# stoyannk/voxels

Hardware: NVIDIA B200
Metric: Mvoxels/s polygonized (higher is better)
Workload: dtype int8 samples / fp32 vertices

## Files before the change

### voxels_b200/csrc/vxb_cell.h

```cpp
#pragma once
#include <stdint.h>

#if defined(__CUDACC__)
#define VXB_FN __device__ __forceinline__
#define VXB_FN_BIG __device__ __forceinline__
#define VXB_SQRT(x) __fsqrt_rn(x)
#define VXB_DIV(a, b) __fdiv_rn((a), (b))
#else
#include <cmath>
#define VXB_FN inline
#define VXB_FN_BIG inline
#define VXB_SQRT(x) std::sqrt(x)
#define VXB_DIV(a, b) ((a) / (b))
#endif

#define VXB_BLOCK 16
#define VXB_EMPTY_MATERIAL 255
#define VXB_NO_SLOT 0xF

enum { VXB_ZPOS = 0, VXB_YPOS = 1, VXB_XPOS = 2, VXB_ZNEG = 3, VXB_YNEG = 4, VXB_XNEG = 5 };

struct VxbGrid
{
	const signed char* dist;
// ... 20 lines not shown
VXB_FN int vxb_clampi(int v, int lo, int hi) { return v < lo ? lo : (v > hi ? hi : v); }

VXB_FN size_t vxb_index(const VxbGrid& g, int x, int y, int z)
{
	const int m = g.n - 1;
	x = vxb_clampi(x, 0, m); y = vxb_clampi(y, 0, m); z = vxb_clampi(z, 0, m);
	return ((size_t)z * g.n + y) * g.n + x;
}

VXB_FN int vxb_dist(const VxbGrid& g, int x, int y, int z) { return g.dist[vxb_index(g, x, y, z)]; }

struct VxbTileView
{
	const signed char* dist;
	const unsigned char* mat;
	const unsigned char* blend;
	int ox, oy, oz;
	int sx, sy, sz;
	int n;
};

VXB_FN int vxb_dist(const VxbTileView& g, int x, int y, int z)
{
	const int xi = (x < g.sx ? g.sx : x) - g.sx, yi = (y < g.sy ? g.sy : y) - g.sy, zi = (z < g.sz ? g.sz : z) - g.sz;
	return g.dist[(zi * 19 + yi) * 48 + xi];
}
VXB_FN size_t vxb_tile_mat_index(const VxbTileView& g, int x, int y, int z)
{
	const int m = g.n - 1;
	return ((size_t)(z > m ? m : z) * g.n + (y > m ? m : y)) * g.n + (x > m ? m : x);
}
VXB_FN unsigned vxb_mat(const VxbTileView& g, int x, int y, int z) { return g.mat[vxb_tile_mat_index(g, x, y, z)]; }
VXB_FN unsigned vxb_blend(const VxbTileView& g, int x, int y, int z) { return g.blend[vxb_tile_mat_index(g, x, y, z)]; }
VXB_FN unsigned vxb_mat(const VxbGrid& g, int x, int y, int z) { return g.mat[vxb_index(g, x, y, z)]; }
VXB_FN unsigned vxb_blend(const VxbGrid& g, int x, int y, int z) { return g.blend[vxb_index(g, x, y, z)]; }

VXB_FN unsigned vxb_case_code(const signed char v[8])
{
	unsigned code = 0;
#pragma unroll
	for (int i = 0; i < 8; ++i) code |= (v[i] < 0 ? 1u : 0u) << i;
	return code;
}

VXB_FN void vxb_normalize_fix_zero(float& x, float& y, float& z)
{
	const float len = VXB_SQRT((x * x + y * y) + z * z);
	if (len <= 1.1920928955078125e-07f) { x = 0.f; y = 0.f; z = 0.f; return; }
	x = VXB_DIV(x, len); y = VXB_DIV(y, len); z = VXB_DIV(z, len);
}

VXB_FN_BIG void vxb_normal(const VxbGrid& g, int x, int y, int z, float n[3])
{
	const int m = g.n - 1;
	const size_t nn = (size_t)g.n;
	const size_t x0 = (size_t)vxb_clampi(x - 1, 0, m), x1 = (size_t)vxb_clampi(x, 0, m), x2 = (size_t)vxb_clampi(x + 1, 0, m);
	const size_t y0 = (size_t)vxb_clampi(y - 1, 0, m) * nn, y1 = (size_t)vxb_clampi(y, 0, m) * nn, y2 = (size_t)vxb_clampi(y + 1, 0, m) * nn;
	const size_t z0 = (size_t)vxb_clampi(z - 1, 0, m) * nn * nn, z1 = (size_t)vxb_clampi(z, 0, m) * nn * nn, z2 = (size_t)vxb_clampi(z + 1, 0, m) * nn * nn;
	const signed char* d = g.dist;
	const int ax = d[z1 + y1 + x2], bx = d[z1 + y1 + x0];
	const int az = d[z2 + y1 + x1], bz = d[z0 + y1 + x1];
	const int ay = d[z1 + y2 + x1], by = d[z1 + y0 + x1];
	n[0] = (float)(ax - bx) * 0.5f;
	n[1] = (float)(az - bz) * 0.5f;
	n[2] = (float)(ay - by) * 0.5f;
	vxb_normalize_fix_zero(n[0], n[1], n[2]);
}

VXB_FN void vxb_normal(const VxbTileView& g, int x, int y, int z, float n[3])
{
	n[0] = (float)(vxb_dist(g, x + 1, y, z) - vxb_dist(g, x - 1, y, z)) * 0.5f;
	n[1] = (float)(vxb_dist(g, x, y, z + 1) - vxb_dist(g, x, y, z - 1)) * 0.5f;
	n[2] = (float)(vxb_dist(g, x, y + 1, z) - vxb_dist(g, x, y - 1, z)) * 0.5f;
	vxb_normalize_fix_zero(n[0], n[1], n[2]);
}

VXB_FN int vxb_fixed_t(int a, int b)
{
#if defined(__CUDA_ARCH__)
	return __float2int_rz(__fdiv_rn((float)(b * 256), (float)(b - a)));
#else
	return (b * 256) / (b - a);
#endif
}

template <class G>
VXB_FN_BIG int vxb_lod_descent(const G& g, int steps, int p0[3], int p1[3])
{
	for (int s = 0; s < steps; ++s)
	{
		const int mx = p0[0] + (p1[0] - p0[0]) / 2, my = p0[1] + (p1[1] - p0[1]) / 2, mz = p0[2] + (p1[2] - p0[2]) / 2;
		const int mid = vxb_dist(g, mx, my, mz);
		const int v0 = vxb_dist(g, p0[0], p0[1], p0[2]);
		if (v0 * mid <= 0) { p1[0] = mx; p1[1] = my; p1[2] = mz; }
		else { p0[0] = mx; p0[1] = my; p0[2] = mz; }
	}
	const int a = vxb_dist(g, p0[0], p0[1], p0[2]);
	const int b = vxb_dist(g, p1[0], p1[1], p1[2]);
	return (a != b) ? vxb_fixed_t(a, b) : 0;
}

VXB_FN unsigned vxb_blend_u8(float f) { return (unsigned)((int)f) & 0xFFu; }

VXB_FN int vxb_corner_flags(int level, int lx, int ly, int lz, int corner)
{
	if (level == 0) return 0;
	int r = 0;
	if (lx == 0 && !(corner & 1)) r |= 1 << VXB_XNEG;
// ... 35 lines not shown

VXB_FN VxbVertexDesc vxb_regular_vertex_desc_lite(unsigned vd, unsigned zeroMask)
{
	VxbVertexDesc d;
	d.v0 = (vd >> 4) & 0xF;
	d.v1 = vd & 0xF;
	d.dir = (vd >> 12) & 0xF;
	d.slot = (vd >> 8) & 0xF;
	const bool z0 = (zeroMask >> d.v0) & 1u, z1 = (zeroMask >> d.v1) & 1u;
	d.endpoint = z0 || z1;
	d.atC7 = false;
	d.t = -1;
	if (d.endpoint)
	{
		d.t = z1 ? 0 : 256;
		d.atC7 = (z1 && d.v1 == 7);
		if (!d.atC7) d.dir = (z1 ? d.v1 : d.v0) ^ 7;
		d.slot = 0;
	}
	return d;
}

VXB_FN VxbVertexDesc vxb_regular_vertex_desc(unsigned vd, const signed char v[8])
{
	VxbVertexDesc d = vxb_regular_vertex_desc_lite(vd, vxb_zero_mask(v));
	if (!d.endpoint) d.t = vxb_fixed_t(v[d.v0], v[d.v1]);
	return d;
}

VXB_FN int vxb_regular_owned_slot(const VxbVertexDesc& d)
{
	if (d.endpoint) return d.atC7 ? 0 : -1;
	return (d.dir == 8) ? d.slot : -1;
}

struct VxbRawVertex
{
	float p[3];
	float s[3];
	float n[3];
	int flags;
	unsigned matId, blend;
};

template <class G>
VXB_FN_BIG void vxb_corner_vertex(const G& g, int level, const int base[3], const int local[3], int corner,
	unsigned cellMatId, unsigned cellMatBlend, VxbRawVertex& out)
{
	const int m = 1 << level;
	const int px = base[0] + ((corner & 1) ? m : 0), py = base[1] + ((corner & 2) ? m : 0), pz = base[2] + ((corner & 4) ? m : 0);
	const unsigned myId = vxb_mat(g, px, py, pz), myBlend = vxb_blend(g, px, py, pz);
	vxb_normal(g, px, py, pz, out.n);
	out.matId = cellMatId;
	out.blend = (myId != cellMatId) ? cellMatBlend : myBlend;
	out.p[0] = (float)px * 256.f; out.p[1] = (float)py * 256.f; out.p[2] = (float)pz * 256.f;
	out.flags = vxb_corner_flags(level, local[0], local[1], local[2], corner);
}

template <class G>
VXB_FN_BIG void vxb_edge_vertex(const G& g, int level, const int base[3], const int local[3], const VxbVertexDesc& d,
	unsigned cellMatId, unsigned cellMatBlend, VxbRawVertex& out)
{
	const int m = 1 << level;
	int p0[3] = { base[0] + ((d.v0 & 1) ? m : 0), base[1] + ((d.v0 & 2) ? m : 0), base[2] + ((d.v0 & 4) ? m : 0) };
	int p1[3] = { base[0] + ((d.v1 & 1) ? m : 0), base[1] + ((d.v1 & 2) ? m : 0), base[2] + ((d.v1 & 4) ? m : 0) };
	int t = d.t;
// ... 261 lines not shown
```

### voxels_b200/csrc/vxb_emit.cuh

```cuda
#pragma once
#ifndef VXB_OCC
#define VXB_OCC 5
#endif
#ifndef VXB_FLAT_OCC
#define VXB_FLAT_OCC 4
#endif
#ifndef VXB_VB_OCC
#define VXB_VB_OCC 8
#endif

template <int PITCH, int ROWS>
__device__ __forceinline__ void vxb_classify_bits(const signed char* tile, unsigned int* rowSign, unsigned int* nt32)
{
	const int tid = threadIdx.x, nthreads = (int)blockDim.x;
	for (int r = tid; r < 17 * 17; r += nthreads)
	{
		const unsigned int* w = reinterpret_cast<const unsigned int*>(tile + ((r / 17) * ROWS + (r % 17)) * PITCH);
		unsigned m = 0;
#pragma unroll
		for (int q = 0; q < 4; ++q) m |= ((((w[q] >> 7) & 0x01010101u) * 0x01020408u) >> 24 & 0xFu) << (4 * q);
		m |= ((w[4] >> 7) & 1u) << 16;
		rowSign[r] = m;
	}
	__syncthreads();
	for (int t = tid; t < 256; t += nthreads)
	{
		const int z = t >> 4, y = t & 15;
		const unsigned a = rowSign[z * 17 + y], b = rowSign[z * 17 + y + 1], c = rowSign[(z + 1) * 17 + y], e = rowSign[(z + 1) * 17 + y + 1];
		const unsigned any = a | b | c | e, all = a & b & c & e;
		reinterpret_cast<unsigned short*>(nt32)[t] = (unsigned short)((any | (any >> 1)) & ~(all & (all >> 1)) & 0xFFFFu);
	}
}

template <int PITCH, int ROWS>
__device__ __forceinline__ void vxb_tile_samples(const signed char* tile, int c, signed char v[8])
{
	const int lx = c & 15, ly = (c >> 4) & 15, lz = c >> 8;
	const signed char* p = tile + (lz * ROWS + ly) * PITCH + lx;
	v[0] = p[0]; v[1] = p[1]; v[2] = p[PITCH]; v[3] = p[PITCH + 1];
	p += ROWS * PITCH;
	v[4] = p[0]; v[5] = p[1]; v[6] = p[PITCH]; v[7] = p[PITCH + 1];
}

__device__ __forceinline__ void vxb_init_cache_page(const VxbDev& d, int level, unsigned coordId)
{
	unsigned int* page = reinterpret_cast<unsigned int*>(d.cachePages[level] + (size_t)coordId * 4096);
	for (int i = threadIdx.x; i < 2048; i += (int)blockDim.x) page[i] = 0x00FF00FFu;
}

__device__ __forceinline__ unsigned vxb_rank_of(const unsigned int* nt32, const unsigned int* wpre, int c)
{
	return wpre[c >> 5] + __popc(nt32[c >> 5] & ((1u << (c & 31)) - 1u));
}

#define VXB_DTILE_PITCH 48
#define VXB_DTILE_BYTES (19 * 19 * VXB_DTILE_PITCH)
template <int MODE, int T> struct VxbBlockCaps { static constexpr int CAP = 1024, VL = (MODE == 0 ? 2048 : 8), NBUF = (MODE == 0 ? 1 : 2); };
template <> struct VxbBlockCaps<0, 128> { static constexpr int CAP = 512, VL = 1024, NBUF = 1; };

template <int MODE, int T>
struct __align__(128) VxbBlockSmem
{
	typedef VxbBlockCaps<MODE, T> Caps;
	signed char tiles[Caps::NBUF][MODE == 0 ? (VXB_DTILE_BYTES + 80) : (VXB_TILE_BYTES + 96)];
	unsigned int rowSign[17 * 17 + 3];
	unsigned int nt32[128];
	unsigned int wpre[132];
	unsigned char tabClass[256];
	unsigned char tabCell[256];
	unsigned short tabVert[3072];
	unsigned int warpSums[8];
	unsigned int hist[16];
	unsigned int used[8];
	unsigned long long mbar[2];
	unsigned int item, hasChild, pageReady, emitIdx, voff, ioff, cellBase, slot, take, removed;
	unsigned int levelEnd[VXB_MAX_LEVELS + 1];
	unsigned int recA[Caps::CAP];
	unsigned int recB[Caps::CAP];
	unsigned short list[Caps::CAP];
	unsigned short cz[Caps::CAP];
	unsigned short vbase[Caps::CAP];
	unsigned short tbase[Caps::CAP];
	unsigned short vl[Caps::VL];
};

__device__ __forceinline__ bool vxb_overflowed(const VxbDev& d)
{
	const VxbCounters* c = d.counters;
	return c->vertices > d.vcap || c->indices > d.icap || c->cells > d.ccap || c->records > d.rcap;
}

template <int MODE, int T>
__global__ void __launch_bounds__(T, (MODE == 0 ? (T == 128 ? 5 : 4) : (MODE == 2 ? 4 : VXB_OCC))) vxb_block_kernel(const __grid_constant__ CUtensorMap tmapA, const __grid_constant__ CUtensorMap tmapB, const VxbDev d, const int levelArg)
{
	constexpr int PITCH = (MODE == 0) ? VXB_DTILE_PITCH : VXB_TILE_PITCH;
	constexpr int ROWS = (MODE == 0) ? 19 : 17;
	typedef VxbBlockSmem<MODE, T> Smem;
	constexpr int CAP_C = Smem::Caps::CAP, VL_CAP = Smem::Caps::VL, NBUF = Smem::Caps::NBUF;
	static_assert(T == 128 || T == 256, "the per-word steps assume 128 or 256 threads");
	extern __shared__ __align__(128) unsigned char smemRaw[];
	Smem& s = *reinterpret_cast<Smem*>(smemRaw);
	const int tid = threadIdx.x;
	const VxbGrid g = d.grid;
	unsigned phaseBits = 0;
	if (tid == 0) { vxb_mbar_init(&s.mbar[0], 1); vxb_mbar_init(&s.mbar[1], 1); }
	if (tid < 16) s.hist[tid] = 0;
	if (tid < 8) s.used[tid] = 0;
	for (int i = tid; i < 256; i += T) { s.tabClass[i] = vxbGRegularCellClass[i]; s.tabCell[i] = vxbGRegularCellData[i]; }
	for (int i = tid; i < 3072; i += T) s.tabVert[i] = vxbGRegularVertexData[i];
	unsigned statNonTrivial = 0;

	unsigned workCount;
	const unsigned* worklist = nullptr;
	unsigned* cursor;
	if (MODE == 2)
	{
		if (tid == 0)
// ... 35 lines not shown
			level = levelArg;
			const int nbl = (d.n >> 4) >> level, sh = __ffs(nbl) - 1;
			const unsigned c = worklist[item];
			bx = c & (nbl - 1); by = (c >> sh) & (nbl - 1); bz = c >> (2 * sh);
		}
	};
	auto issue = [&](int buf, int level, int bx, int by, int bz) {
		if (MODE == 0)
		{
			if (tid == 0)
			{
				const int sx = bx ? bx * 16 - 16 : 0, sy = by ? by * 16 - 1 : 0, sz = bz ? bz * 16 - 1 : 0;
				vxb_fence_proxy_async();
				vxb_mbar_expect_tx(&s.mbar[buf], VXB_DTILE_BYTES);
				vxb_tma_load_3d(s.tiles[buf], &tmapA, sx, sy, sz, &s.mbar[buf]);
			}
		}
		else if (MODE == 1) vxb_tile_issue(s.tiles[buf], &s.mbar[buf], &tmapA, &tmapB, d, level, bx, by, bz);
	};

	if (tid == 0) s.item = atomicAdd(cursor, 1u);
	__syncthreads();
	unsigned item = s.item;
	int buf = 0;
	if (item < workCount) { int l, x, y, z; decode(item, l, x, y, z); issue(0, l, x, y, z); }
	__syncthreads();

	while (item < workCount)
	{
		if (tid == 0) { s.item = atomicAdd(cursor, 1u); s.hasChild = 0; s.pageReady = 0; s.take = 1; s.removed = 0; }
		__syncthreads();
		const unsigned nextItem = s.item;
		bool nextIssued = false;
		if (nextItem < workCount && MODE != 2 && NBUF == 2) { int l, x, y, z; decode(nextItem, l, x, y, z); issue(buf ^ 1, l, x, y, z); nextIssued = true; }
		int level, bx, by, bz;
		decode(item, level, bx, by, bz);
		const int m = 1 << level, nb = d.n / 16 / m;
		const unsigned coordId = ((unsigned)bz * nb + by) * nb + bx;
		const bool midLevel = level > 0 && level != d.lastLevel;
		signed char* const tileRaw = s.tiles[(MODE == 2 || NBUF == 1) ? 0 : buf];

		if (MODE == 2)
		{
			if (tid < 32)
			{
				const int cnb = nb * 2, cl = level - 1;
				if (level > d.coarseLo && tid < 8)
				{
					const int cx = bx * 2 + (tid & 1), cy = by * 2 + ((tid >> 1) & 1), cz = bz * 2 + (tid >> 2);
					const bool inRun = !(d.ranged && (cx < d.rangeMin[cl][0] || cx >= d.rangeMax[cl][0] || cy < d.rangeMin[cl][1] || cy >= d.rangeMax[cl][1] || cz < d.rangeMin[cl][2] || cz >= d.rangeMax[cl][2]));
					if (inRun)
					{
						const volatile unsigned char* flag = d.coarseDone + d.coarseBase[cl] + ((size_t)cz * cnb + cy) * cnb + cx;
						unsigned spins = 0;
						while (!*flag) { __nanosleep(32); if (++spins > (1u << 24)) __trap(); }
					}
					__threadfence();
				}
				__syncwarp();
				unsigned u = 0, anyChild = 0;
				if (tid < 27)
				{
					const int x = tid % 3, y = (tid / 3) % 3, z = tid / 9;
					const int cx = min(2 * bx + x, cnb - 1), cy = min(2 * by + y, cnb - 1), cz = min(2 * bz + z, cnb - 1);
					const size_t cb = ((size_t)cz * cnb + cy) * cnb + cx;
					u = d.mixInfo[cl][cb];
// ... 44 lines not shown
				__syncthreads();
				for (int i = tid; i < 19 * VXB_DTILE_PITCH; i += T)
				{
					const int z = i / VXB_DTILE_PITCH, x = i % VXB_DTILE_PITCH;
					signed char* p = tileRaw + z * 19 * VXB_DTILE_PITCH + x;
					for (int q = lastY + 1; q < 19; ++q) p[q * VXB_DTILE_PITCH] = p[lastY * VXB_DTILE_PITCH];
				}
			}
			if (bz == nb - 1)
			{
				__syncthreads();
				for (int i = tid; i < 19 * VXB_DTILE_PITCH; i += T)
				{
					const int y = i / VXB_DTILE_PITCH, x = i % VXB_DTILE_PITCH;
					signed char* p = tileRaw + y * VXB_DTILE_PITCH + x;
					for (int q = lastZ + 1; q < 19; ++q) p[q * 19 * VXB_DTILE_PITCH] = p[lastZ * 19 * VXB_DTILE_PITCH];
				}
			}
			tile = tileRaw + ((bz * 16 - hsz) * 19 + (by * 16 - hsy)) * VXB_DTILE_PITCH + (bx * 16 - hsx);
		}
		else if (MODE == 2)
		{
			vxb_mbar_wait(&s.mbar[0], phaseBits & 1u);
			phaseBits ^= 1u;
			tile = tileRaw;
		}
		else
		{
			unsigned ph = (phaseBits >> buf) & 1u;
			vxb_tile_complete(tileRaw, &s.mbar[buf], ph, d, level, bx, by, bz);
			phaseBits = (phaseBits & ~(1u << buf)) | (ph << buf);
			tile = tileRaw;
		}
		__syncthreads();

		vxb_classify_bits<PITCH, ROWS>(tile, s.rowSign, s.nt32);
		__syncthreads();
		unsigned ntc;
		{
			const unsigned cnt = (tid < 128) ? __popc(s.nt32[tid]) : 0u;
			const unsigned ex = vxb_block_scan(cnt, s.warpSums, ntc);
			if (tid < 128) s.wpre[tid] = ex;
		}
		__syncthreads();
		const bool inCap = ntc <= (unsigned)CAP_C;
		const bool emitMine = MODE != 2 || vxb_coarse_emit_is_mine(d, level, coordId);

		if (ntc > 0)
		{
			if (level == 0)
			{
				if (tid < 128)
				{
					unsigned* page = d.consPages + (size_t)coordId * 128;
					page[tid] = d.consValid[coordId] ? (page[tid] | s.nt32[tid]) : s.nt32[tid];
				}
			}
			else if (!d.cacheValid[level][coordId]) vxb_init_cache_page(d, level, coordId);
			if (inCap)
			{
				for (int r = tid; r < 256; r += T)
				{
					unsigned bits = reinterpret_cast<const unsigned short*>(s.nt32)[r];
					unsigned pos = s.wpre[r >> 1] + ((r & 1) ? __popc(s.nt32[r >> 1] & 0xFFFFu) : 0u);
					while (bits) { const int x = __ffs(bits) - 1; bits &= bits - 1; s.list[pos++] = (unsigned short)(r * 16 + x); }
				}
			}
			__syncthreads();
			if (tid == 0)
			{
				if (level == 0) d.consValid[coordId] = 1; else d.cacheValid[level][coordId] = 1;
				s.pageReady = 1;
				if (emitMine)
				{
					const unsigned idx = d.workBase[level] + atomicAdd(&d.counters->emitCount[level], 1u);
					d.emitList[idx] = ((unsigned)level << 28) | coordId;
					s.emitIdx = idx;
					statNonTrivial += ntc;
				}
			}
			auto cellWork = [&](int c) {
				signed char v[8];
				vxb_tile_samples<PITCH, ROWS>(tile, c, v);
				if (emitMine) atomicAdd(&s.hist[s.tabClass[vxb_case_code(v)]], 1u);
				if (level > 0)
				{
					const VxbVoteSource voteSrc = vxb_vote_source(d, level);
					const int vote = vxb_vote_cell(voteSrc, (bx * 16 + (c & 15)) * m, (by * 16 + ((c >> 4) & 15)) * m, (bz * 16 + (c >> 8)) * m);
					if (vote >= 0) d.cachePages[level][(size_t)coordId * 4096 + c] = (unsigned short)vote;
				}
			};
			if (inCap) { if (level > 0) for (unsigned i = tid; i < ntc; i += T) cellWork(s.list[i]); }
			else
			{
				for (int r = tid; r < 256; r += T)
				{
					unsigned bits = reinterpret_cast<const unsigned short*>(s.nt32)[r];
					while (bits) { const int x = __ffs(bits) - 1; bits &= bits - 1; cellWork(r * 16 + x); }
				}
			}
			__syncthreads();
			if (!inCap && emitMine && tid < 128) { d.ntScratch[(size_t)s.emitIdx * 256 + tid] = s.nt32[tid]; d.ntScratch[(size_t)s.emitIdx * 256 + 128 + tid] = s.wpre[tid]; }
		}

		if (MODE != 0 && midLevel)
		{
			const VxbVoteSource voteSrc = vxb_vote_source(d, level);
			if (tid < 8)
			{
				const int cnb = nb * 2;
				const size_t cb = ((size_t)(bz * 2 + (tid >> 2)) * cnb + (by * 2 + ((tid >> 1) & 1))) * cnb + (bx * 2 + (tid & 1));
				const bool valid = (level == 1) ? __ldcg(d.consValid + cb) : __ldcg(d.cacheValid[level - 1] + cb);
				if (valid) atomicOr(&s.hasChild, 1u);
			}
			__syncthreads();
			if (s.hasChild)
			{
				if (!s.pageReady)
				{
					if (!d.cacheValid[level][coordId]) vxb_init_cache_page(d, level, coordId);
					__syncthreads();
					if (tid == 0) { d.cacheValid[level][coordId] = 1; s.pageReady = 1; }
				}
				for (int fc = tid; fc < 256; fc += T)
				{
				const int row = fc >> 4, col = fc & 15;
				unsigned candidates = 0;
#pragma unroll
				for (int face = 0; face < 6; ++face)
				{
					int axis, ua, va;
					vxb_face_axes(face, axis, ua, va);
					const int bc = (axis == 0) ? bx : (axis == 1 ? by : bz);
					const bool outside = face < 3 ? (bc == 0) : (bc == nb - 1);
					const int edge = (face >= 3) ? 15 : 0;
					const int lx = axis == 0 ? edge : col, ly = axis == 1 ? edge : (axis == 2 ? row : col), lz = axis == 2 ? edge : row;
					if (vxb_vote_candidate(voteSrc, (bx * 16 + lx) * m, (by * 16 + ly) * m, (bz * 16 + lz) * m) && !outside) candidates |= 1u << face;
				}
				while (candidates)
				{
					const int face = __ffs(candidates) - 1;
					candidates &= candidates - 1;
					int axis, ua, va;
					vxb_face_axes(face, axis, ua, va);
					const int edge = (face >= 3) ? 15 : 0;
					const int local[3] = { axis == 0 ? edge : col, axis == 1 ? edge : (axis == 2 ? row : col), axis == 2 ? edge : row };
					const int vote = vxb_vote_cell(voteSrc, (bx * 16 + local[0]) * m, (by * 16 + local[1]) * m, (bz * 16 + local[2]) * m);
					if (vote >= 0) d.cachePages[level][(size_t)coordId * 4096 + local[2] * 256 + local[1] * 16 + local[0]] = (unsigned short)vote;
				}
				}
			}
		}
		__syncthreads();
		if (MODE == 2 && tid == 0) { __threadfence(); *(volatile unsigned char*)(d.coarseDone + d.coarseBase[level] + coordId) = 1; }

		if (ntc > 0 && !inCap)
		{
			if (tid == 0 && emitMine) d.bigList[atomicAdd(&d.counters->bigCount[0], 1u)] = s.emitIdx;
		}
		else if (ntc > 0 && emitMine)
		{
			for (unsigned i = tid; i < ntc; i += T)
			{
				const int c = s.list[i];
				signed char v[8];
				vxb_tile_samples<PITCH, ROWS>(tile, c, v);
				const unsigned code = vxb_case_code(v);
				const unsigned zm = vxb_zero_mask(v);
				unsigned matId, matBlend;
				if (level == 0)
				{
					atomicAdd(&s.hist[s.tabClass[code]], 1u);
					const size_t gi = ((size_t)((bz * 16 + (c >> 8))) * d.n + (by * 16 + ((c >> 4) & 15))) * d.n + (bx * 16 + (c & 15));
					matId = g.mat[gi]; matBlend = g.blend[gi];
				}
				else
				{
					const unsigned e = d.cachePages[level][(size_t)coordId * 4096 + c];
					matId = e & 0xFF; matBlend = e >> 8;
				}
				unsigned slotK = 0xFFFFu;
				const int nv = s.tabCell[s.tabClass[code] * 16] >> 4;
				for (int k = 0; k < nv; ++k)
				{
					const VxbVertexDesc vd = vxb_regular_vertex_desc_lite(s.tabVert[code * 12 + k], zm);
					const int sl = vxb_regular_owned_slot(vd);
					if (sl >= 0) slotK = (slotK & ~(0xFu << (4 * sl))) | ((unsigned)k << (4 * sl));
				}
				s.cz[i] = (unsigned short)(code | (zm << 8));
				s.recA[i] = matId | (matBlend << 8) | (slotK << 16);
			}
			__syncthreads();

			for (unsigned i = tid; i < ntc; i += T)
			{
				const int c = s.list[i];
				const unsigned code = s.cz[i] & 0xFF, zm = s.cz[i] >> 8;
				const unsigned geo = s.tabCell[s.tabClass[code] * 16];
				const unsigned rowStart = vxb_rank_of(s.nt32, s.wpre, c & ~15), sliceStart = s.wpre[(c >> 8) * 8];
				const int mask = (i > rowStart ? 1 : 0) | (rowStart > sliceStart ? 2 : 0) | (sliceStart > 0 ? 4 : 0);
				const unsigned myMat = s.recA[i] & 0xFF;
				unsigned newMask = 0, quirkMask = 0;
				for (int k = 0; k < (int)(geo >> 4); ++k)
				{
					const VxbVertexDesc vd = vxb_regular_vertex_desc_lite(s.tabVert[code * 12 + k], zm);
					bool isNew = true;
					if (!vd.atC7 && (vd.dir & mask) == vd.dir)
					{
						const int oc = c - (vd.dir & 1) - ((vd.dir >> 1) & 1) * 16 - ((vd.dir >> 2) & 1) * 256;
						int ok = VXB_NO_SLOT; unsigned oa = 0;
						if ((s.nt32[oc >> 5] >> (oc & 31)) & 1u)
						{
							oa = s.recA[vxb_rank_of(s.nt32, s.wpre, oc)];
							ok = (oa >> (16 + 4 * vd.slot)) & 0xF;
						}
						if (ok != VXB_NO_SLOT) { if ((oa & 0xFF) == myMat) isNew = false; }
						else if (vd.endpoint) quirkMask |= 1u << k;
					}
					if (isNew) newMask |= 1u << k;
				}
				s.recB[i] = newMask | (quirkMask << 12) | ((unsigned)mask << 24);
				s.vbase[i] = (unsigned short)__popc(newMask);
				s.tbase[i] = (unsigned short)(geo & 0xF);
			}
			__syncthreads();

			unsigned nverts, ntris;
			{
				const unsigned per = (ntc + T - 1) / T;
				const unsigned i0 = min(tid * per, ntc), i1 = min(i0 + per, ntc);
				unsigned sv = 0, st = 0;
				for (unsigned i = i0; i < i1; ++i) { sv += s.vbase[i]; st += s.tbase[i]; }
				unsigned total;
				const unsigned base = vxb_block_scan(sv | (st << 16), s.warpSums, total);
				nverts = total & 0xFFFF; ntris = total >> 16;
				unsigned bv = base & 0xFFFF, bt = base >> 16;
				for (unsigned i = i0; i < i1; ++i)
				{
					const unsigned cv = s.vbase[i], ct = s.tbase[i];
					s.vbase[i] = (unsigned short)bv; s.tbase[i] = (unsigned short)bt;
					bv += cv; bt += ct;
				}
			}
			const bool inCta = MODE == 0 && nverts <= (unsigned)VL_CAP;
			if (MODE == 0 && !inCta)
			{
				__syncthreads();
				if (tid < 128) { d.ntScratch[(size_t)s.emitIdx * 256 + tid] = s.nt32[tid]; d.ntScratch[(size_t)s.emitIdx * 256 + 128 + tid] = s.wpre[tid]; }
				if (tid == 0) d.bigList[atomicAdd(&d.counters->bigCount[0], 1u)] = s.emitIdx;
			}
			else
			{
				if (tid == 0) s.voff = atomicAdd(&d.counters->vertices, nverts);
				if (tid == 32) s.ioff = atomicAdd(&d.counters->indices, ntris * 3);
				if (tid == 64) s.cellBase = (MODE == 0) ? 0u : atomicAdd(&d.counters->cells, ntc);
				if (tid == 96) s.slot = atomicAdd(&d.counters->records, 1u);
				__syncthreads();
				const unsigned voff = s.voff, ioff = s.ioff, cellBase = s.cellBase, slot = s.slot;
				const bool fits = (unsigned long long)voff + nverts <= d.vcap && (unsigned long long)ioff + ntris * 3ull <= d.icap
					&& (unsigned long long)cellBase + ntc <= d.ccap && slot < d.rcap;
				if (fits && MODE != 0)
				{
					for (unsigned i = tid; i < ntc; i += T)
					{
						const unsigned rb = s.recB[i];
						VxbCellRec cr;
						cr.a = (unsigned)s.list[i] | ((unsigned)s.cz[i] << 12) | ((rb >> 24) << 28);
						cr.b = s.recA[i];
						cr.c = rb & 0x00FFFFFFu;
						cr.d = (unsigned)s.vbase[i] | ((unsigned)s.tbase[i] << 16);
						*reinterpret_cast<uint4*>(&d.cellRecs[cellBase + i]) = *reinterpret_cast<const uint4*>(&cr);
						d.cellBlock[cellBase + i] = slot;
						unsigned nm = rb & 0xFFFu, j = voff + s.vbase[i];
						while (nm) { const int k = __ffs(nm) - 1; nm &= nm - 1; d.vlist[j++] = ((cellBase + i) << 4) | (unsigned)k; }
					}
					if (tid < 128) { d.ntScratch[(size_t)s.emitIdx * 256 + tid] = s.nt32[tid]; d.ntScratch[(size_t)s.emitIdx * 256 + 128 + tid] = s.wpre[tid]; }
				}
				if (fits && MODE == 0)
				{
					for (unsigned i = tid; i < ntc; i += T)
					{
						unsigned nm = s.recB[i] & 0xFFFu, j = s.vbase[i];
						while (nm) { const int k = __ffs(nm) - 1; nm &= nm - 1; s.vl[j++] = (unsigned short)((i << 4) | (unsigned)k); }
					}
					__syncthreads();
					VxbTileView tv;
					tv.dist = tileRaw; tv.ox = bx * 16; tv.oy = by * 16; tv.oz = bz * 16; tv.sx = hsx; tv.sy = hsy; tv.sz = hsz;
					tv.mat = g.mat; tv.blend = g.blend; tv.n = d.n;
					for (unsigned j = tid; j < nverts; j += T)
					{
						const unsigned e = s.vl[j];
						const unsigned i = e >> 4; const int k = e & 15;
						const int c = s.list[i];
						const unsigned code = s.cz[i] & 0xFF, zm = s.cz[i] >> 8;
						const int local[3] = { c & 15, (c >> 4) & 15, c >> 8 };
						const int base[3] = { bx * 16 + local[0], by * 16 + local[1], bz * 16 + local[2] };
						const unsigned ra = s.recA[i];
						const unsigned matId = ra & 0xFF, matBlend = (ra >> 8) & 0xFF;
						VxbVertexDesc vd = vxb_regular_vertex_desc_lite(s.tabVert[code * 12 + k], zm);
						VxbRawVertex rv;
						if (vd.endpoint)
						{
							const bool quirk = (s.recB[i] >> (12 + k)) & 1u;
							vxb_corner_vertex(tv, 0, base, local, quirk ? vd.v0 : ((vd.t == 0) ? vd.v1 : vd.v0), matId, matBlend, rv);
						}
						else
						{
							const int a = vxb_dist(tv, base[0] + (vd.v0 & 1), base[1] + ((vd.v0 >> 1) & 1), base[2] + (vd.v0 >> 2));
							const int b = vxb_dist(tv, base[0] + (vd.v1 & 1), base[1] + ((vd.v1 >> 1) & 1), base[2] + (vd.v1 >> 2));
							vd.t = vxb_fixed_t(a, b);
							vxb_edge_vertex(tv, 0, base, local, vd, matId, matBlend, rv);
						}
						vxb_regular_secondary(0, rv);
						VxbVertex ov;
						vxb_finish_vertex(rv, *d.lut, ov);
						vxb_store_vertex(d.verts + voff + j, ov);
						atomicOr(&s.used[matId >> 5], 1u << (matId & 31));
					}
					__syncthreads();
					if (NBUF == 1 && nextItem < workCount) { int l2, x2, y2, z2; decode(nextItem, l2, x2, y2, z2); issue(0, l2, x2, y2, z2); nextIssued = true; }
					unsigned removed = 0;
					for (unsigned i = tid; i < ntc; i += T)
					{
						const int c = s.list[i];
						const unsigned code = s.cz[i] & 0xFF, zm = s.cz[i] >> 8;
						const unsigned char* cd = &s.tabCell[s.tabClass[code] * 16];
						const unsigned geo = cd[0];
						const unsigned newMask = s.recB[i] & 0xFFFu;
						unsigned w[6] = { 0u, 0u, 0u, 0u, 0u, 0u };
						unsigned nextNew = s.vbase[i];
						const int nv = (int)(geo >> 4);
#pragma unroll
						for (int k = 0; k < 12; ++k)
						{
							if (k < nv)
							{
								unsigned vid;
								if ((newMask >> k) & 1u) vid = nextNew++;
								else
								{
									const VxbVertexDesc vd = vxb_regular_vertex_desc_lite(s.tabVert[code * 12 + k], zm);
									const int oc = c - (vd.dir & 1) - ((vd.dir >> 1) & 1) * 16 - ((vd.dir >> 2) & 1) * 256;
									const unsigned oi = vxb_rank_of(s.nt32, s.wpre, oc);
									const unsigned ok = (s.recA[oi] >> (16 + 4 * vd.slot)) & 0xF;
									vid = (unsigned)s.vbase[oi] + __popc(s.recB[oi] & 0xFFFu & ((1u << ok) - 1u));
								}
								w[k >> 1] |= vid << ((k & 1) * 16);
							}
						}
						auto vidOf = [&](unsigned k) -> unsigned {
							const unsigned q = k >> 1;
							const unsigned pair = q == 0 ? w[0] : q == 1 ? w[1] : q == 2 ? w[2] : q == 3 ? w[3] : q == 4 ? w[4] : w[5];
							return (k & 1u) ? (pair >> 16) : (pair & 0xFFFFu);
						};
						unsigned* out = d.idx + ioff + (unsigned)s.tbase[i] * 3;
						const bool cannotDegenerate = zm == 0u;
						for (unsigned tr = 0; tr < (geo & 0xF); ++tr, out += 3)
						{
							const unsigned a = vidOf(cd[1 + tr * 3]), b = vidOf(cd[2 + tr * 3]), cc = vidOf(cd[3 + tr * 3]);
							bool kept = true;
							if (!cannotDegenerate)
							{
								const float* fa = d.verts[voff + a].pos; const float* fb = d.verts[voff + b].pos; const float* fc = d.verts[voff + cc].pos;
								const float pa[3] = { fa[0] * 256.f, fa[2] * 256.f, fa[1] * 256.f };
								const float pb[3] = { fb[0] * 256.f, fb[2] * 256.f, fb[1] * 256.f };
								const float pc[3] = { fc[0] * 256.f, fc[2] * 256.f, fc[1] * 256.f };
								kept = vxb_triangle_kept(pa, pb, pc);
							}
							if (kept) { out[0] = a; out[1] = b; out[2] = cc; }
							else { out[0] = 0xFFFFFFFFu; out[1] = 0xFFFFFFFFu; out[2] = 0xFFFFFFFFu; ++removed; }
						}
					}
					if (removed) atomicAdd(&s.removed, removed);
					__syncthreads();
				}
				if (fits && tid == 0)
				{
					VxbBlockRec br;
					br.packed = ((unsigned)level << 28) | coordId; br.emitIdx = s.emitIdx; br.voff = voff; br.ioff = ioff; br.cellBase = cellBase;
					br.ntc = ntc; br.nverts = nverts; br.ntris = ntris; br.removed = (MODE == 0) ? s.removed : 0u;
					for (int f = 0; f < 6; ++f) { br.tvoff[f] = 0; br.tioff[f] = 0; br.tvcount[f] = 0; br.ticount[f] = 0; }
					br.pad[0] = br.pad[1] = br.pad[2] = 0;
					d.blockRecs[slot] = br;
					if (level > 0 && level != d.lastLevel && d.transitions) d.transList[atomicAdd(&d.counters->transBlocks, 1u)] = slot;
				}
			}
		}
		__syncthreads();
		if (NBUF == 1 && MODE != 2 && !nextIssued && nextItem < workCount) { int l2, x2, y2, z2; decode(nextItem, l2, x2, y2, z2); issue(0, l2, x2, y2, z2); }
		item = nextItem;
		if (NBUF == 2) buf ^= 1;
	}

	__syncthreads();
	if (tid < 16 && s.hist[tid]) atomicAdd(&d.counters->perCase[tid], s.hist[tid]);
	if (tid < 8 && s.used[tid]) atomicOr(&d.counters->usedMaterials[tid], s.used[tid]);
	if (tid == 0 && statNonTrivial) atomicAdd(&d.counters->nonTrivial, statNonTrivial);
}

template <int CAP_C>
struct __align__(128) VxbDecideSmem
{
	signed char tile[VXB_TILE_BYTES + 96];
	unsigned int nt32[128];
	unsigned int wpre[132];
	unsigned char tabClass[256];
	unsigned char tabCell[256];
	unsigned short tabVert[3072];
	unsigned int warpSums[8];
	unsigned long long mbar;
	unsigned int item, voff, ioff, cellBase, slot;
	unsigned int levelEnd[VXB_MAX_LEVELS + 1];
	unsigned int recA[CAP_C];
	unsigned int recB[CAP_C];
	unsigned short list[CAP_C];
	unsigned short cz[CAP_C];
	unsigned short vbase[CAP_C];
	unsigned short tbase[CAP_C];
};

template <int CAP_C, int TIER>
// ... 798 lines not shown
```

### voxels_b200/csrc/vxb_kernels.cuh

```cuda
#pragma once

#define VXB_MAX_LEVELS 12
#define VXB_THREADS 256
#define VXB_TILE_PITCH 32
#define VXB_TILE_BYTES (17 * 17 * VXB_TILE_PITCH)

#define VXB_BI_NEG 1u
#define VXB_BI_NONNEG 2u
#define VXB_BI_EMPTY 4u
#define VXB_BI_NEG_E 8u
#define VXB_BI_NONNEG_E 16u

struct VxbCounters
{
	unsigned int vertices, indices, transVertices, transIndices;
	unsigned int records;
	unsigned int nonSkippedLevel0;
	unsigned int nonTrivial;
	unsigned int degenerate;
	unsigned int perCase[16];
	unsigned int usedMaterials[8];
	unsigned int workCount[VXB_MAX_LEVELS];
	unsigned int workCursor[VXB_MAX_LEVELS];
	unsigned int emitCount[VXB_MAX_LEVELS];
// ... 107 lines not shown
__device__ __forceinline__ void vxb_mbar_expect_tx(unsigned long long* bar, unsigned bytes)
{
	asm volatile("mbarrier.arrive.expect_tx.shared::cta.b64 _, [%0], %1;" ::"r"(vxb_smem_addr(bar)), "r"(bytes) : "memory");
}

__device__ __forceinline__ void vxb_mbar_wait(unsigned long long* bar, unsigned parity)
{
	const unsigned addr = vxb_smem_addr(bar);
	unsigned done, spins = 0;
	do
	{
		asm volatile(
			"{\n"
			".reg .pred p;\n"
			"mbarrier.try_wait.parity.shared::cta.b64 p, [%1], %2;\n"
			"selp.u32 %0, 1, 0, p;\n"
			"}\n" : "=r"(done) : "r"(addr), "r"(parity) : "memory");
		if (!done && ++spins > (1u << 26)) __trap();
	} while (!done);
}

__device__ __forceinline__ void vxb_tma_load_3d(void* dst, const CUtensorMap* map, int x, int y, int z, unsigned long long* bar)
{
	asm volatile(
		"cp.async.bulk.tensor.3d.shared::cluster.global.tile.mbarrier::complete_tx::bytes [%0], [%1, {%2, %3, %4}], [%5];"
		::"r"(vxb_smem_addr(dst)), "l"(map), "r"(x), "r"(y), "r"(z), "r"(vxb_smem_addr(bar)) : "memory");
}

__device__ __forceinline__ void vxb_fence_proxy_async()
{
	asm volatile("fence.proxy.async.shared::cta;" ::: "memory");
}

__device__ __forceinline__ unsigned vxb_block_scan(unsigned v, unsigned* warpSums , unsigned& total)
{
	const int nwarps = (int)(blockDim.x >> 5);
	const unsigned lane = threadIdx.x & 31, warp = threadIdx.x >> 5;
	unsigned inc = v;
#pragma unroll
	for (int o = 1; o < 32; o <<= 1)
	{
		const unsigned t = __shfl_up_sync(0xFFFFFFFFu, inc, o);
		if (lane >= (unsigned)o) inc += t;
	}
	__syncthreads();
	if (lane == 31) warpSums[warp] = inc;
	__syncthreads();
	unsigned base = 0, tot = 0;
#pragma unroll
	for (int w = 0; w < VXB_THREADS / 32; ++w)
	{
		if (w >= nwarps) break;
		const unsigned s = warpSums[w];
		if ((unsigned)w < warp) base += s;
		tot += s;
	}
	total = tot;
	return base + inc - v;
}

__device__ __forceinline__ unsigned vxb_zero_bytes(unsigned w)
{
	return ~(((w & 0x7F7F7F7Fu) + 0x7F7F7F7Fu) | w) & 0x80808080u;
}

struct VxbCoarseLattices
{
	unsigned char* p[VXB_MAX_LEVELS];
	int lo, levels;
};

__global__ void __launch_bounds__(256) vxb_coarse_lattice_kernel(const signed char* __restrict__ dist, int n, const __grid_constant__ VxbCoarseLattices lat,
	int planesPerPiece, int zOwnerWorld, int zOwnerRank)
{
	const int lane = threadIdx.x & 31;
	const unsigned warpsPerGrid = gridDim.x * (blockDim.x >> 5);
	unsigned w = blockIdx.x * (blockDim.x >> 5) + (threadIdx.x >> 5);
	for (int l = lat.lo; l < lat.levels; ++l)
// ... 696 lines not shown
```

Before: 737,300.

## Streamline level-0 block emission: fused classify, cached vertex decode, fewer barriers

Result: faster. 785,300 (median of 6 runs) (+6.5%).

```diff
diff --git a/voxels_b200/csrc/vxb_cell.h b/voxels_b200/csrc/vxb_cell.h
--- a/voxels_b200/csrc/vxb_cell.h
+++ b/voxels_b200/csrc/vxb_cell.h
@@ -76,6 +76,12 @@
 }
 VXB_FN unsigned vxb_mat(const VxbTileView& g, int x, int y, int z) { return g.mat[vxb_tile_mat_index(g, x, y, z)]; }
 VXB_FN unsigned vxb_blend(const VxbTileView& g, int x, int y, int z) { return g.blend[vxb_tile_mat_index(g, x, y, z)]; }
+
+struct VxbTileViewInterior : VxbTileView {};
+VXB_FN int vxb_dist(const VxbTileViewInterior& g, int x, int y, int z) { return g.dist[((z - g.sz) * 19 + (y - g.sy)) * 48 + (x - g.sx)]; }
+VXB_FN size_t vxb_tile_mat_index(const VxbTileViewInterior& g, int x, int y, int z) { return ((size_t)z * g.n + y) * g.n + x; }
+VXB_FN unsigned vxb_mat(const VxbTileViewInterior& g, int x, int y, int z) { return g.mat[vxb_tile_mat_index(g, x, y, z)]; }
+VXB_FN unsigned vxb_blend(const VxbTileViewInterior& g, int x, int y, int z) { return g.blend[vxb_tile_mat_index(g, x, y, z)]; }
 VXB_FN unsigned vxb_mat(const VxbGrid& g, int x, int y, int z) { return g.mat[vxb_index(g, x, y, z)]; }
 VXB_FN unsigned vxb_blend(const VxbGrid& g, int x, int y, int z) { return g.blend[vxb_index(g, x, y, z)]; }
 
@@ -111,13 +117,16 @@
 	vxb_normalize_fix_zero(n[0], n[1], n[2]);
 }
 
-VXB_FN void vxb_normal(const VxbTileView& g, int x, int y, int z, float n[3])
+template <class TV>
+VXB_FN void vxb_tile_normal(const TV& g, int x, int y, int z, float n[3])
 {
 	n[0] = (float)(vxb_dist(g, x + 1, y, z) - vxb_dist(g, x - 1, y, z)) * 0.5f;
 	n[1] = (float)(vxb_dist(g, x, y, z + 1) - vxb_dist(g, x, y, z - 1)) * 0.5f;
 	n[2] = (float)(vxb_dist(g, x, y + 1, z) - vxb_dist(g, x, y - 1, z)) * 0.5f;
 	vxb_normalize_fix_zero(n[0], n[1], n[2]);
 }
+VXB_FN void vxb_normal(const VxbTileView& g, int x, int y, int z, float n[3]) { vxb_tile_normal(g, x, y, z, n); }
+VXB_FN void vxb_normal(const VxbTileViewInterior& g, int x, int y, int z, float n[3]) { vxb_tile_normal(g, x, y, z, n); }
 
 VXB_FN int vxb_fixed_t(int a, int b)
 {
@@ -219,6 +228,11 @@
 {
 	if (d.endpoint) return d.atC7 ? 0 : -1;
 	return (d.dir == 8) ? d.slot : -1;
+}
+
+VXB_FN unsigned vxb_regular_reuse_code(const VxbVertexDesc& d)
+{
+	return ((d.atC7 || d.dir == 8) ? 0u : (unsigned)d.dir) | ((unsigned)d.slot << 3);
 }
 
 struct VxbRawVertex
diff --git a/voxels_b200/csrc/vxb_emit.cuh b/voxels_b200/csrc/vxb_emit.cuh
--- a/voxels_b200/csrc/vxb_emit.cuh
+++ b/voxels_b200/csrc/vxb_emit.cuh
@@ -10,26 +10,22 @@
 #endif
 
 template <int PITCH, int ROWS>
-__device__ __forceinline__ void vxb_classify_bits(const signed char* tile, unsigned int* rowSign, unsigned int* nt32)
-{
-	const int tid = threadIdx.x, nthreads = (int)blockDim.x;
-	for (int r = tid; r < 17 * 17; r += nthreads)
-	{
-		const unsigned int* w = reinterpret_cast<const unsigned int*>(tile + ((r / 17) * ROWS + (r % 17)) * PITCH);
-		unsigned m = 0;
+__device__ __forceinline__ unsigned vxb_row_sign(const signed char* tile, int z, int y)
+{
+	const unsigned int* w = reinterpret_cast<const unsigned int*>(tile + (z * ROWS + y) * PITCH);
+	unsigned m = 0;
 #pragma unroll
-		for (int q = 0; q < 4; ++q) m |= ((((w[q] >> 7) & 0x01010101u) * 0x01020408u) >> 24 & 0xFu) << (4 * q);
-		m |= ((w[4] >> 7) & 1u) << 16;
-		rowSign[r] = m;
-	}
-	__syncthreads();
-	for (int t = tid; t < 256; t += nthreads)
-	{
-		const int z = t >> 4, y = t & 15;
-		const unsigned a = rowSign[z * 17 + y], b = rowSign[z * 17 + y + 1], c = rowSign[(z + 1) * 17 + y], e = rowSign[(z + 1) * 17 + y + 1];
-		const unsigned any = a | b | c | e, all = a & b & c & e;
-		reinterpret_cast<unsigned short*>(nt32)[t] = (unsigned short)((any | (any >> 1)) & ~(all & (all >> 1)) & 0xFFFFu);
-	}
+	for (int q = 0; q < 4; ++q) m |= ((((w[q] >> 7) & 0x01010101u) * 0x01020408u) >> 24 & 0xFu) << (4 * q);
+	return m | ((w[4] >> 7) & 1u) << 16;
+}
+template <int PITCH, int ROWS>
+__device__ __forceinline__ unsigned vxb_row_nontrivial(const signed char* tile, int r)
+{
+	const int z = r >> 4, y = r & 15;
+	const unsigned a = vxb_row_sign<PITCH, ROWS>(tile, z, y), b = vxb_row_sign<PITCH, ROWS>(tile, z, y + 1);
+	const unsigned c = vxb_row_sign<PITCH, ROWS>(tile, z + 1, y), e = vxb_row_sign<PITCH, ROWS>(tile, z + 1, y + 1);
+	const unsigned any = a | b | c | e, all = a & b & c & e;
+	return (any | (any >> 1)) & ~(all & (all >> 1)) & 0xFFFFu;
 }
 
 template <int PITCH, int ROWS>
@@ -63,7 +59,6 @@
 {
 	typedef VxbBlockCaps<MODE, T> Caps;
 	signed char tiles[Caps::NBUF][MODE == 0 ? (VXB_DTILE_BYTES + 80) : (VXB_TILE_BYTES + 96)];
-	unsigned int rowSign[17 * 17 + 3];
 	unsigned int nt32[128];
 	unsigned int wpre[132];
 	unsigned char tabClass[256];
@@ -82,7 +77,9 @@
 	unsigned short vbase[Caps::CAP];
 	unsigned short tbase[Caps::CAP];
 	unsigned short vl[Caps::VL];
+	unsigned long long vdec[MODE == 0 ? Caps::CAP : 1];
 };
+static_assert(sizeof(VxbBlockSmem<0, 256>) + 1024 <= 228 * 1024 / 4, "level-0 block kernel no longer fits 4 CTAs per SM");
 
 __device__ __forceinline__ bool vxb_overflowed(const VxbDev& d)
 {
@@ -184,6 +181,7 @@
 		__syncthreads();
 		const unsigned nextItem = s.item;
 		bool nextIssued = false;
+		unsigned removedSlot = ~0u;
 		if (nextItem < workCount && MODE != 2 && NBUF == 2) { int l, x, y, z; decode(nextItem, l, x, y, z); issue(buf ^ 1, l, x, y, z); nextIssued = true; }
 		int level, bx, by, bz;
 		decode(item, level, bx, by, bz);
@@ -294,17 +292,17 @@
 			phaseBits = (phaseBits & ~(1u << buf)) | (ph << buf);
 			tile = tileRaw;
 		}
-		__syncthreads();
-
-		vxb_classify_bits<PITCH, ROWS>(tile, s.rowSign, s.nt32);
-		__syncthreads();
-		unsigned ntc;
-		{
-			const unsigned cnt = (tid < 128) ? __popc(s.nt32[tid]) : 0u;
-			const unsigned ex = vxb_block_scan(cnt, s.warpSums, ntc);
-			if (tid < 128) s.wpre[tid] = ex;
-		}
-		__syncthreads();
+		if (MODE != 0 || bx == nb - 1 || by == nb - 1 || bz == nb - 1) __syncthreads();
+
+		constexpr int ROWS_PER_THREAD = 256 / T;
+		unsigned ntc, rowPre, rowBits;
+		{
+			if (T == 256) reinterpret_cast<unsigned short*>(s.nt32)[tid] = (unsigned short)(rowBits = vxb_row_nontrivial<PITCH, ROWS>(tile, tid));
+			else s.nt32[tid] = rowBits = vxb_row_nontrivial<PITCH, ROWS>(tile, 2 * tid) | vxb_row_nontrivial<PITCH, ROWS>(tile, 2 * tid + 1) << 16;
+			rowPre = vxb_block_scan<false>(__popc(rowBits), s.warpSums, ntc);
+			if (ROWS_PER_THREAD == 2) s.wpre[tid] = rowPre;
+			else if ((tid & 1) == 0) s.wpre[tid >> 1] = rowPre;
+		}
 		const bool inCap = ntc <= (unsigned)CAP_C;
 		const bool emitMine = MODE != 2 || vxb_coarse_emit_is_mine(d, level, coordId);
 
@@ -321,12 +319,8 @@
 			else if (!d.cacheValid[level][coordId]) vxb_init_cache_page(d, level, coordId);
 			if (inCap)
 			{
-				for (int r = tid; r < 256; r += T)
-				{
-					unsigned bits = reinterpret_cast<const unsigned short*>(s.nt32)[r];
-					unsigned pos = s.wpre[r >> 1] + ((r & 1) ? __popc(s.nt32[r >> 1] & 0xFFFFu) : 0u);
-					while (bits) { const int x = __ffs(bits) - 1; bits &= bits - 1; s.list[pos++] = (unsigned short)(r * 16 + x); }
-				}
+				unsigned bits = rowBits, pos = rowPre;
+				while (bits) { const int x = __ffs(bits) - 1; bits &= bits - 1; s.list[pos++] = (unsigned short)(tid * 16 * ROWS_PER_THREAD + x); }
 			}
 			__syncthreads();
 			if (tid == 0)
@@ -361,7 +355,7 @@
 					while (bits) { const int x = __ffs(bits) - 1; bits &= bits - 1; cellWork(r * 16 + x); }
 				}
 			}
-			__syncthreads();
+			if (MODE != 0 || !inCap) __syncthreads();
 			if (!inCap && emitMine && tid < 128) { d.ntScratch[(size_t)s.emitIdx * 256 + tid] = s.nt32[tid]; d.ntScratch[(size_t)s.emitIdx * 256 + 128 + tid] = s.wpre[tid]; }
 		}
 
@@ -413,7 +407,7 @@
 				}
 			}
 		}
-		__syncthreads();
+		if (MODE != 0) __syncthreads();
 		if (MODE == 2 && tid == 0) { __threadfence(); *(volatile unsigned char*)(d.coarseDone + d.coarseBase[level] + coordId) = 1; }
 
 		if (ntc > 0 && !inCap)
@@ -442,13 +436,15 @@
 					matId = e & 0xFF; matBlend = e >> 8;
 				}
 				unsigned slotK = 0xFFFFu;
+				unsigned long long dec = 0;
 				const int nv = s.tabCell[s.tabClass[code] * 16] >> 4;
 				for (int k = 0; k < nv; ++k)
 				{
-					const VxbVertexDesc vd = vxb_regular_vertex_desc_lite(s.tabVert[code * 12 + k], zm);
-					const int sl = vxb_regular_owned_slot(vd);
-					if (sl >= 0) slotK = (slotK & ~(0xFu << (4 * sl))) | ((unsigned)k << (4 * sl));
-				}
+					const unsigned rc = vxb_regular_reuse_code(vxb_regular_vertex_desc_lite(s.tabVert[code * 12 + k], zm));
+					if ((rc & 7u) == 0u) slotK = (slotK & ~(0xFu << (4 * (rc >> 3)))) | ((unsigned)k << (4 * (rc >> 3)));
+					dec |= (unsigned long long)rc << (5 * k);
+				}
+				if (MODE == 0) s.vdec[i] = dec;
 				s.cz[i] = (unsigned short)(code | (zm << 8));
 				s.recA[i] = matId | (matBlend << 8) | (slotK << 16);
 			}
@@ -459,25 +455,28 @@
 				const int c = s.list[i];
 				const unsigned code = s.cz[i] & 0xFF, zm = s.cz[i] >> 8;
 				const unsigned geo = s.tabCell[s.tabClass[code] * 16];
+				const unsigned long long dec = (MODE == 0) ? s.vdec[i] : 0ull;
 				const unsigned rowStart = vxb_rank_of(s.nt32, s.wpre, c & ~15), sliceStart = s.wpre[(c >> 8) * 8];
 				const int mask = (i > rowStart ? 1 : 0) | (rowStart > sliceStart ? 2 : 0) | (sliceStart > 0 ? 4 : 0);
 				const unsigned myMat = s.recA[i] & 0xFF;
 				unsigned newMask = 0, quirkMask = 0;
 				for (int k = 0; k < (int)(geo >> 4); ++k)
 				{
-					const VxbVertexDesc vd = vxb_regular_vertex_desc_lite(s.tabVert[code * 12 + k], zm);
+					const unsigned rc = (MODE == 0) ? (unsigned)(dec >> (5 * k)) & 31u
+						: vxb_regular_reuse_code(vxb_regular_vertex_desc_lite(s.tabVert[code * 12 + k], zm));
+					const unsigned dir = rc & 7u, slot = rc >> 3;
 					bool isNew = true;
-					if (!vd.atC7 && (vd.dir & mask) == vd.dir)
+					if (dir != 0u && (dir & mask) == dir)
 					{
-						const int oc = c - (vd.dir & 1) - ((vd.dir >> 1) & 1) * 16 - ((vd.dir >> 2) & 1) * 256;
+						const int oc = c - (dir & 1) - ((dir >> 1) & 1) * 16 - ((dir >> 2) & 1) * 256;
 						int ok = VXB_NO_SLOT; unsigned oa = 0;
 						if ((s.nt32[oc >> 5] >> (oc & 31)) & 1u)
 						{
 							oa = s.recA[vxb_rank_of(s.nt32, s.wpre, oc)];
-							ok = (oa >> (16 + 4 * vd.slot)) & 0xF;
+							ok = (oa >> (16 + 4 * slot)) & 0xF;
 						}
 						if (ok != VXB_NO_SLOT) { if ((oa & 0xFF) == myMat) isNew = false; }
-						else if (vd.endpoint) quirkMask |= 1u << k;
+						else if (slot == 0u) quirkMask |= 1u << k;
 					}
 					if (isNew) newMask |= 1u << k;
 				}
@@ -494,13 +493,19 @@
 				unsigned sv = 0, st = 0;
 				for (unsigned i = i0; i < i1; ++i) { sv += s.vbase[i]; st += s.tbase[i]; }
 				unsigned total;
-				const unsigned base = vxb_block_scan(sv | (st << 16), s.warpSums, total);
+				const unsigned base = vxb_block_scan<false>(sv | (st << 16), s.warpSums, total);
 				nverts = total & 0xFFFF; ntris = total >> 16;
 				unsigned bv = base & 0xFFFF, bt = base >> 16;
+				const bool writeVl = MODE == 0 && nverts <= (unsigned)VL_CAP;
 				for (unsigned i = i0; i < i1; ++i)
 				{
 					const unsigned cv = s.vbase[i], ct = s.tbase[i];
 					s.vbase[i] = (unsigned short)bv; s.tbase[i] = (unsigned short)bt;
+					if (writeVl)
+					{
+						unsigned nm = s.recB[i] & 0xFFFu, j = bv;
+						while (nm) { const int k = __ffs(nm) - 1; nm &= nm - 1; s.vl[j++] = (unsigned short)((i << 4) | (unsigned)k); }
+					}
 					bv += cv; bt += ct;
 				}
 			}
@@ -540,88 +545,73 @@
 				}
 				if (fits && MODE == 0)
 				{
-					for (unsigned i = tid; i < ntc; i += T)
-					{
-						unsigned nm = s.recB[i] & 0xFFFu, j = s.vbase[i];
-						while (nm) { const int k = __ffs(nm) - 1; nm &= nm - 1; s.vl[j++] = (unsigned short)((i << 4) | (unsigned)k); }
-					}
-					__syncthreads();
 					VxbTileView tv;
 					tv.dist = tileRaw; tv.ox = bx * 16; tv.oy = by * 16; tv.oz = bz * 16; tv.sx = hsx; tv.sy = hsy; tv.sz = hsz;
 					tv.mat = g.mat; tv.blend = g.blend; tv.n = d.n;
-					for (unsigned j = tid; j < nverts; j += T)
+					auto vertexPass = [&](const auto& view) {
+						for (unsigned j = tid; j < nverts; j += T)
+						{
+							const unsigned e = s.vl[j];
+							const unsigned i = e >> 4; const int k = e & 15;
+							const int c = s.list[i];
+							const unsigned code = s.cz[i] & 0xFF;
+							const int local[3] = { c & 15, (c >> 4) & 15, c >> 8 };
+							const int base[3] = { bx * 16 + local[0], by * 16 + local[1], bz * 16 + local[2] };
+							const unsigned ra = s.recA[i];
+							const unsigned matId = ra & 0xFF, matBlend = (ra >> 8) & 0xFF;
+							const unsigned rc = (unsigned)(s.vdec[i] >> (5 * k)) & 31u, raw = s.tabVert[code * 12 + k];
+							VxbVertexDesc vd;
+							vd.v0 = (raw >> 4) & 0xF; vd.v1 = raw & 0xF; vd.dir = rc & 7; vd.slot = rc >> 3;
+							vd.endpoint = vd.slot == 0; vd.atC7 = false; vd.t = -1;
+							VxbRawVertex rv;
+							if (vd.endpoint)
+							{
+								const bool quirk = (s.recB[i] >> (12 + k)) & 1u;
+								vxb_corner_vertex(view, 0, base, local, quirk ? vd.v0 : (vd.dir ^ 7), matId, matBlend, rv);
+							}
+							else
+							{
+								const int a = vxb_dist(view, base[0] + (vd.v0 & 1), base[1] + ((vd.v0 >> 1) & 1), base[2] + (vd.v0 >> 2));
+								const int b = vxb_dist(view, base[0] + (vd.v1 & 1), base[1] + ((vd.v1 >> 1) & 1), base[2] + (vd.v1 >> 2));
+								vd.t = vxb_fixed_t(a, b);
+								vxb_edge_vertex(view, 0, base, local, vd, matId, matBlend, rv);
+							}
+							vxb_regular_secondary(0, rv);
+							VxbVertex ov;
+							vxb_finish_vertex(rv, *d.lut, ov);
+							vxb_store_vertex(d.verts + voff + j, ov);
+							atomicOr(&s.used[matId >> 5], 1u << (matId & 31));
+						}
+					};
+					if (bx > 0 && by > 0 && bz > 0 && bx < nb - 1 && by < nb - 1 && bz < nb - 1)
 					{
-						const unsigned e = s.vl[j];
-						const unsigned i = e >> 4; const int k = e & 15;
+						VxbTileViewInterior ti;
+						static_cast<VxbTileView&>(ti) = tv;
+						vertexPass(ti);
+					}
+					else vertexPass(tv);
+
+					unsigned removed = 0;
+					auto cellTriangles = [&](unsigned i, bool testDegenerate) {
 						const int c = s.list[i];
-						const unsigned code = s.cz[i] & 0xFF, zm = s.cz[i] >> 8;
-						const int local[3] = { c & 15, (c >> 4) & 15, c >> 8 };
-						const int base[3] = { bx * 16 + local[0], by * 16 + local[1], bz * 16 + local[2] };
-						const unsigned ra = s.recA[i];
-						const unsigned matId = ra & 0xFF, matBlend = (ra >> 8) & 0xFF;
-						VxbVertexDesc vd = vxb_regular_vertex_desc_lite(s.tabVert[code * 12 + k], zm);
-						VxbRawVertex rv;
-						if (vd.endpoint)
-						{
-							const bool quirk = (s.recB[i] >> (12 + k)) & 1u;
-							vxb_corner_vertex(tv, 0, base, local, quirk ? vd.v0 : ((vd.t == 0) ? vd.v1 : vd.v0), matId, matBlend, rv);
-						}
-						else
-						{
-							const int a = vxb_dist(tv, base[0] + (vd.v0 & 1), base[1] + ((vd.v0 >> 1) & 1), base[2] + (vd.v0 >> 2));
-							const int b = vxb_dist(tv, base[0] + (vd.v1 & 1), base[1] + ((vd.v1 >> 1) & 1), base[2] + (vd.v1 >> 2));
-							vd.t = vxb_fixed_t(a, b);
-							vxb_edge_vertex(tv, 0, base, local, vd, matId, matBlend, rv);
-						}
-						vxb_regular_secondary(0, rv);
-						VxbVertex ov;
-						vxb_finish_vertex(rv, *d.lut, ov);
-						vxb_store_vertex(d.verts + voff + j, ov);
-						atomicOr(&s.used[matId >> 5], 1u << (matId & 31));
-					}
-					__syncthreads();
-					if (NBUF == 1 && nextItem < workCount) { int l2, x2, y2, z2; decode(nextItem, l2, x2, y2, z2); issue(0, l2, x2, y2, z2); nextIssued = true; }
-					unsigned removed = 0;
-					for (unsigned i = tid; i < ntc; i += T)
-					{
-						const int c = s.list[i];
-						const unsigned code = s.cz[i] & 0xFF, zm = s.cz[i] >> 8;
-						const unsigned char* cd = &s.tabCell[s.tabClass[code] * 16];
+						const unsigned char* cd = &s.tabCell[s.tabClass[s.cz[i] & 0xFF] * 16];
 						const unsigned geo = cd[0];
-						const unsigned newMask = s.recB[i] & 0xFFFu;
-						unsigned w[6] = { 0u, 0u, 0u, 0u, 0u, 0u };
-						unsigned nextNew = s.vbase[i];
-						const int nv = (int)(geo >> 4);
-#pragma unroll
-						for (int k = 0; k < 12; ++k)
-						{
-							if (k < nv)
-							{
-								unsigned vid;
-								if ((newMask >> k) & 1u) vid = nextNew++;
-								else
-								{
-									const VxbVertexDesc vd = vxb_regular_vertex_desc_lite(s.tabVert[code * 12 + k], zm);
-									const int oc = c - (vd.dir & 1) - ((vd.dir >> 1) & 1) * 16 - ((vd.dir >> 2) & 1) * 256;
-									const unsigned oi = vxb_rank_of(s.nt32, s.wpre, oc);
-									const unsigned ok = (s.recA[oi] >> (16 + 4 * vd.slot)) & 0xF;
-									vid = (unsigned)s.vbase[oi] + __popc(s.recB[oi] & 0xFFFu & ((1u << ok) - 1u));
-								}
-								w[k >> 1] |= vid << ((k & 1) * 16);
-							}
-						}
+						const unsigned newMask = s.recB[i] & 0xFFFu, vb = s.vbase[i];
+						const unsigned long long dec = s.vdec[i];
 						auto vidOf = [&](unsigned k) -> unsigned {
-							const unsigned q = k >> 1;
-							const unsigned pair = q == 0 ? w[0] : q == 1 ? w[1] : q == 2 ? w[2] : q == 3 ? w[3] : q == 4 ? w[4] : w[5];
-							return (k & 1u) ? (pair >> 16) : (pair & 0xFFFFu);
+							if ((newMask >> k) & 1u) return vb + __popc(newMask & ((1u << k) - 1u));
+							const unsigned rc = (unsigned)(dec >> (5 * k)) & 31u, dir = rc & 7u;
+							const int oc = c - (dir & 1) - ((dir >> 1) & 1) * 16 - ((dir >> 2) & 1) * 256;
+							const unsigned oi = vxb_rank_of(s.nt32, s.wpre, oc);
+							const unsigned ok = (s.recA[oi] >> (16 + 4 * (rc >> 3))) & 0xF;
+							return (unsigned)s.vbase[oi] + __popc(s.recB[oi] & 0xFFFu & ((1u << ok) - 1u));
 						};
-						unsigned* out = d.idx + ioff + (unsigned)s.tbase[i] * 3;
-						const bool cannotDegenerate = zm == 0u;
+					unsigned* out = d.idx + ioff + (unsigned)s.tbase[i] * 3;
 						for (unsigned tr = 0; tr < (geo & 0xF); ++tr, out += 3)
 						{
 							const unsigned a = vidOf(cd[1 + tr * 3]), b = vidOf(cd[2 + tr * 3]), cc = vidOf(cd[3 + tr * 3]);
 							bool kept = true;
-							if (!cannotDegenerate)
+							if (testDegenerate)
 							{
 								const float* fa = d.verts[voff + a].pos; const float* fb = d.verts[voff + b].pos; const float* fc = d.verts[voff + cc].pos;
 								const float pa[3] = { fa[0] * 256.f, fa[2] * 256.f, fa[1] * 256.f };
@@ -632,15 +622,21 @@
 							if (kept) { out[0] = a; out[1] = b; out[2] = cc; }
 							else { out[0] = 0xFFFFFFFFu; out[1] = 0xFFFFFFFFu; out[2] = 0xFFFFFFFFu; ++removed; }
 						}
-					}
+					};
+					for (unsigned i = T - 1 - tid; i < ntc; i += T)
+						if ((s.cz[i] >> 8) == 0u) cellTriangles(i, false);
+					__syncthreads();
+					if (NBUF == 1 && nextItem < workCount) { int l2, x2, y2, z2; decode(nextItem, l2, x2, y2, z2); issue(0, l2, x2, y2, z2); nextIssued = true; }
+					for (unsigned i = T - 1 - tid; i < ntc; i += T)
+						if ((s.cz[i] >> 8) != 0u) cellTriangles(i, true);
 					if (removed) atomicAdd(&s.removed, removed);
-					__syncthreads();
+					if (tid == 0) removedSlot = slot;
 				}
 				if (fits && tid == 0)
 				{
 					VxbBlockRec br;
 					br.packed = ((unsigned)level << 28) | coordId; br.emitIdx = s.emitIdx; br.voff = voff; br.ioff = ioff; br.cellBase = cellBase;
-					br.ntc = ntc; br.nverts = nverts; br.ntris = ntris; br.removed = (MODE == 0) ? s.removed : 0u;
+					br.ntc = ntc; br.nverts = nverts; br.ntris = ntris; br.removed = 0;
 					for (int f = 0; f < 6; ++f) { br.tvoff[f] = 0; br.tioff[f] = 0; br.tvcount[f] = 0; br.ticount[f] = 0; }
 					br.pad[0] = br.pad[1] = br.pad[2] = 0;
 					d.blockRecs[slot] = br;
@@ -649,6 +645,7 @@
 			}
 		}
 		__syncthreads();
+		if (MODE == 0 && tid == 0 && removedSlot != ~0u && s.removed) d.blockRecs[removedSlot].removed = s.removed;
 		if (NBUF == 1 && MODE != 2 && !nextIssued && nextItem < workCount) { int l2, x2, y2, z2; decode(nextItem, l2, x2, y2, z2); issue(0, l2, x2, y2, z2); }
 		item = nextItem;
 		if (NBUF == 2) buf ^= 1;
diff --git a/voxels_b200/csrc/vxb_kernels.cuh b/voxels_b200/csrc/vxb_kernels.cuh
--- a/voxels_b200/csrc/vxb_kernels.cuh
+++ b/voxels_b200/csrc/vxb_kernels.cuh
@@ -163,6 +163,7 @@
 	asm volatile("fence.proxy.async.shared::cta;" ::: "memory");
 }
 
+template <bool LEAD_SYNC = true>
 __device__ __forceinline__ unsigned vxb_block_scan(unsigned v, unsigned* warpSums , unsigned& total)
 {
 	const int nwarps = (int)(blockDim.x >> 5);
@@ -174,7 +175,7 @@
 		const unsigned t = __shfl_up_sync(0xFFFFFFFFu, inc, o);
 		if (lane >= (unsigned)o) inc += t;
 	}
-	__syncthreads();
+	if (LEAD_SYNC) __syncthreads();
 	if (lane == 31) warpSums[warp] = inc;
 	__syncthreads();
 	unsigned base = 0, tot = 0;
```
